# dubhater/vapoursynth-mvtools

Measured on AMD Instinct MI355X. Metric: MDegrain3 cfg3 fps (Super+Analyse+Degrain end-to-end), higher is better.
Workload: dtype u16; 1 GPU; 4K YUV420P16 Degrain3 blksize=16 overlap=8 pel=2; batches_in_flight=2

## Files before the change

### vapoursynth-mvtools_amd/csrc/mvx_analyse.hip

```cpp
#include <stdarg.h>
#include <stdlib.h>

#include <algorithm>
#include "mvx_analyse_kernel.h"
#include "mvx_analyse_fast.h"
#include "mvx_analyse_spec.h"
int mvx_analyse_launch_spec_u8(const AParams &P, const ASpecLaunch &S);
int mvx_analyse_launch_spec_u16(const AParams &P, const ASpecLaunch &S);


static thread_local char g_err[512];
void mvx_set_error(const char *fmt, ...) {
    va_list ap;
    va_start(ap, fmt);
    vsnprintf(g_err, sizeof(g_err), fmt, ap);
    va_end(ap);
}
extern "C" __attribute__((visibility("default"))) const char *mvx_last_error(void) { return g_err; }

struct MvxDebug {
    int general = 0;
    int cpw1 = 0;
    int spec = 1;
    int team = -1;
// ... 278 lines not shown
        int fMaxBlkX = 0;
        for (int i = 0; i < P.nLevels; i++) if (P.lv[i].nBlkX > fMaxBlkX) fMaxBlkX = P.lv[i].nBlkX;
        const int fBins = 1024;
        int fNeed = fRow + fMaxBlkX * 16;
        if (fNeed < fRow + fBins * 4) fNeed = fRow + fBins * 4;
        const bool stripShape8 = P.bps == 1 && P.blkX == 8 && P.chroma && (P.ovX == 4 || P.ovX == 0) && P.shadow[1] != 0;
        const bool uvOrLumaOnly = P.chroma ? P.shadow[1] != 0 : true;
        const bool stripShape16 = P.bps == 1 && P.blkX == 16 && uvOrLumaOnly && (P.ovX == 8 || P.ovX == 0);
        const bool stripShape = (P.bps == 2 && (P.blkX == 16 || (MVX_STRIP32 && P.blkX == 32)) && uvOrLumaOnly && (P.ovX == P.blkX / 2 || (P.blkX == 16 && P.ovX == 0))) || stripShape8 || stripShape16;
        const int sStrip = (P.bps == 2 && P.blkX == 16) ? 2 * 24 * 128  : (P.bps == 2 && MVX_STRIP32 && P.blkX == 32) ? (P.blkX + P.blkX / 2) * 128 : (P.bps == 1 && P.blkX == 16) ? 24 * 64 : 0;
        const int sSrc = stripShape8 ? 16 + 768 : fRow < sStrip ? sStrip : fRow;
        int sNeed = 0, sTabMax = 0;
        for (int i = 0; i < P.nLevels; i++) {
            const bool smallest = i == P.nLevels - 1;
            const int st = smallest ? (P.nLevels == 1 ? P.searchType : P.searchTypeCoarse) : (i == 0 ? P.searchType : P.searchTypeCoarse);
            const int tabB = (st == SearchHex2 ? SPEC_SLOTS_HEX : SPEC_SLOTS_EXH) * SPEC_STRIDE;
            const int need = sSrc + ((P.lv[i].nBlkX * 8 + 15) & ~15) + tabB;
            if (need > sNeed) sNeed = need;
            if (tabB > sTabMax) sTabMax = tabB;
        }
        if (sNeed < sSrc + fBins * 4) sNeed = sSrc + fBins * 4;
        const int teamShared = (64 + fMaxBlkX * 8 + 255) & ~255;
        const int teamPerWave = ((sSrc + sTabMax < sSrc + fBins * 4 ? sSrc + fBins * 4 : sSrc + sTabMax) + 255) & ~255;
        auto teamThatFits = [&](int team) {
            if (team == 1 || team > 8) team = 0;
            while (team > 1 && teamShared + teamPerWave * team > 160 * 1024) team--;
            return team > 1 ? team : 0;
        };
        const bool teamAnyShape = g_dbg.spec == 1 && g_dbg.team < 0 && teamThatFits(mvx_team_default(njobs, simds, false, P.bps)) > 0;
        const bool useSpec = g_dbg.spec != 0 && (stripShape || g_dbg.spec >= 2 || teamAnyShape);
        const bool useSpecStrips = useSpec && g_dbg.spec != 3 && stripShape;
        int sTab = 0, sRow = fRow;
        if (useSpec) {
            sRow = sSrc;
            sTab = sSrc + ((fMaxBlkX * 8 + 15) & ~15);
            fNeed = sNeed;
        }
        const int perChain = (fNeed + 255) & ~255;
        auto have = [&](int k) {
            if (P.bps == 2 && P.blkX == 8) return k == 1 || k == 2 || k == 4;
            if (P.bps == 2 && P.blkX == 32) return k >= 1 && k <= 3;
            return k >= 1 && k <= 4;
        };
        int k = njobs > 3 * simds ? 4 : njobs > 2 * simds ? 3 : njobs > simds ? 2 : 1;
        if (useSpecStrips && k > 2) k = 2;
        while (k > 1 && (!have(k) || (long long)perChain * 4 * k > 160 * 1024)) k--;
        if ((long long)perChain * 4 * k <= 160 * 1024) {
            const int cpw = useSpecStrips ? 4 : 4 * k;
            int syncEvery = k >= 2 ? (P.bps == 2 ? 32 : 256) : 0;
            if (useSpecStrips) syncEvery = (stripShape8 || stripShape16) ? 0 : 128;
            const int flags = MVX_FAST_XCD_REMAP | ((P.shadow[1] != 0 && P.chroma) ? MVX_FAST_UV : 0) | (g_dbg.spec == 2 ? MVX_FAST_NOSPEC : 0) | (g_dbg.spec == 3 ? MVX_FAST_NOSTRIP : 0);
            const ALaunch L = { njobs, 0, useSpec ? sRow : fRow, useSpec ? sRow : fRow, fBins, fNeed, simds, cpw, k, syncEvery, k, flags, st, a->dP, S.d };
            int rc;
            const int specSide = (P.blkX == 16 && P.ovX == 0) ? 1 : 0;
            const int team = useSpec ? teamThatFits(g_dbg.team >= 0 ? g_dbg.team : mvx_team_default(njobs, simds, useSpecStrips, P.bps)) : 0;
            if (team) {
                ALaunch TL = L;
                TL.ldsRow = teamShared; TL.ldsNeed = teamPerWave; TL.ldsHist = sRow; TL.syncEvery = 0; TL.fast = 2; TL.cpw = 1;
                const ASpecLaunch SL = { TL, sRow, team, specSide };
                rc = P.bps == 1 ? mvx_analyse_launch_spec_u8(P, SL) : mvx_analyse_launch_spec_u16(P, SL);
                if (rc == MVX_OK) return finish(2, team, 0, 3);
                if (rc != 1) return rc;
            }
            if (useSpec) { const ASpecLaunch SL = { L, sTab, 0, specSide }; rc = P.bps == 1 ? mvx_analyse_launch_spec_u8(P, SL) : mvx_analyse_launch_spec_u16(P, SL); }
            else rc = P.bps == 1 ? mvx_analyse_launch_fast_u8(P, L) : mvx_analyse_launch_fast_u16(P, L);
            if (rc == MVX_OK) return finish(k, cpw, syncEvery, useSpec ? 2 : 0);
            if (rc != 1) return rc;
        }
    }
    const bool specialised = P.dctmode == 0 && P.xr == 2 && P.yr == 2 && P.blkX == P.blkY && (P.blkX == 16 || P.blkX == 8 || (P.blkX == 32 && P.bps == 2));
    int cpw = g_dbg.cpw1 ? 1 : 4, wpe = 1;
    if (specialised && !g_dbg.cpw1 && njobs > simds) {
        if (P.bps == 1 && (P.blkX == 8 || P.blkX == 16)) wpe = 2;
        if (P.bps == 1 && P.blkX == 8 && njobs > 2 * simds) wpe = 3;
        if (P.bps == 2 && (P.blkX == 16 || P.blkX == 8 || P.blkX == 32)) { wpe = 2; cpw = 8; }
    }
    int srcBytes = P.blkX * P.blkY * P.bps;
    if (P.chroma) srcBytes += 2 * (P.blkX / P.xr) * (P.blkY / P.yr) * P.bps;
    int ldsRow = (srcBytes + 15) & ~15;
    int maxBlkX = 0;
    for (int i = 0; i < P.nLevels; i++) if (P.lv[i].nBlkX > maxBlkX) maxBlkX = P.lv[i].nBlkX;
    const int histBins = 1024;
    const int ldsHist = ldsRow + maxBlkX * 16;
    int ldsBytes = ldsHist + histBins * 4;
    if (ldsBytes > 160 * 1024) { mvx_set_error("mvx_analyse_frames: frame too wide for the LDS row buffer"); return MVX_E_ARG; }
    const int ldsNeed = ldsBytes;
    if (ldsBytes < 33 * 1024) ldsBytes = 33 * 1024;
    while (cpw > 1 && (long long)((ldsNeed + 255) & ~255) * cpw > 160 * 1024) {
        cpw = cpw == 8 ? 4 : 1;
        if (wpe == 3) wpe = 2;
        if (P.bps == 2) wpe = 1;
    }
    const int syncEvery = wpe >= 2 ? 256 : 0;
    const ALaunch L = { njobs, ldsBytes, ldsRow, ldsHist, histBins, ldsNeed, simds, cpw, wpe, syncEvery, 0, 0, st, a->dP, S.d };
    bool off32 = true;
    for (int i = 0; i < P.nLevels; i++)
        if ((long long)P.lv[i].pel * P.lv[i].pel * P.lv[i].pstride[0] >= 0xffffffffLL || (long long)P.lv[i].pel * P.lv[i].pel * P.lv[i].pstride[1] >= 0xffffffffLL) off32 = false;
    int rc = (P.dctmode != 0 || !off32) ? 1 : P.bps == 1 ? mvx_analyse_launch_u8(P, L) : mvx_analyse_launch_u16(P, L);
    if (rc == 1) rc = mvx_analyse_launch_any(P, L);
    if (rc) return rc;
    return finish(0, cpw, syncEvery, 0);
}


struct mvx_recalculate {
    mvx_analysis_data ad, adOut, old;
    AParams P;
// ... 165 lines not shown
```

### vapoursynth-mvtools_amd/csrc/mvx_analyse_spec.h

```cpp
#pragma once
#include <type_traits>
#include "mvx_analyse_fast.h"

#define SPEC_TB 32
#define SPEC_STRIDE (SPEC_TB * 8 + 8)
#define SPEC_SLOTS_HEX 19
#define SPEC_SLOTS_EXH 29
#define MVX_FAST_NOSTRIP 8
#define MVX_FAST_NOSPEC 4

constexpr int SPEC_SW3 = 12;
#ifdef MVX_SPEC_PROF
#define SPROF_N 20
static __device__ unsigned long long g_specprof[SPROF_N];
#define SPROF(i) do { const long long t1_ = (long long)__builtin_amdgcn_s_memtime(); asm volatile("s_waitcnt lgkmcnt(0)" : : "s"(t1_) : "memory"); sprof[i] += t1_ - sprofT; sprofT = t1_; } while (0)
#else
#define SPROF(i) ((void)0)
#endif
#ifdef MVX_SPEC_PROF
#define SPEC_PROF_DUMP_() do { if (l == 0 && chain == 5 && S.role == 1) for (int i = 0; i < SPROF_N; i++) g_specprof[i] = (unsigned long long)S.sprof[i]; } while (0)
#else
#define SPEC_PROF_DUMP_() ((void)0)
#endif
#ifdef MVX_SPEC_STATS
// ... 86 lines not shown
        const unsigned idx = (unsigned)((ax & m) | ((ay & m) << logPel));
        return idx * pstrideC + (unsigned)(ay >> logPel) * pitchC + (unsigned)(ax >> logPel) * BPS;
    }
    template <int LOGG, int WMAX> __device__ __forceinline__ void pass_start(int s, int bx0, int vx, int vy, int vyc, unsigned &oA, unsigned &oB) const {
        typedef PG<LOGG, WMAX> Q;
        const int rowA = s >> G::LLOGC, xbA = (s & (Q::CA - 1)) * G::LCB, rowB = s >> G::UVLOGC, xbB = (s & (Q::CB - 1)) * G::UVCB;
        oA = luma_off_at(bx0, vx, vy) + (unsigned)rowA * pitchY + (unsigned)xbA;
        oB = 2 * chroma_off_at(bx0, vx, vyc) + (unsigned)rowB * 2 * pitchC + (unsigned)xbB;
    }
    template <int LOGG, int WMAX> __device__ __forceinline__ v4u pass_issue(Pass<LOGG, WMAX> &T, int piece) const {
        typedef PG<LOGG, WMAX> Q;
        v4u v;
        if (piece < Q::NA) { v = F::template ld_ref<G::LCB>(refY + T.curA); T.curA += (unsigned)(Q::GG >> G::LLOGC) * pitchY; asm volatile("" : "+v"(T.curA) : : "memory"); }
        else { v = F::template ld_ref<G::UVCB>(refUV + T.curB); T.curB += (unsigned)(Q::GG >> G::UVLOGC) * 2 * pitchC; asm volatile("" : "+v"(T.curB) : : "memory"); }
        return v;
    }
    template <int LOGG, int WMAX> __device__ __forceinline__ void pass_prime(Pass<LOGG, WMAX> &T, unsigned oA, unsigned oB) const {
        typedef PG<LOGG, WMAX> Q;
        T.curA = oA; T.curB = oB;
#pragma unroll
        for (int k = 0; k < Q::W; k++) T.r[k] = pass_issue(T, k);
    }
    template <int LOGG, int WMAX, bool REFILL = true> __device__ __forceinline__ void pass_run(Pass<LOGG, WMAX> &T, int s, unsigned nA, unsigned nB) const {
        typedef PG<LOGG, WMAX> Q;
        const int rowA = s >> G::LLOGC, xbA = (s & (Q::CA - 1)) * G::LCB, rowB = s >> G::UVLOGC, xbB = (s & (Q::CB - 1)) * G::UVCB;
        const lds_u8 *spA = lds + rowA * G::LROWB + xbA, *spB = lds + G::UOFF + rowB * G::UVROWB + xbB;
        constexpr int lstepA = (Q::GG >> G::LLOGC) * G::LROWB, lstepB = (Q::GG >> G::UVLOGC) * G::UVROWB;
        auto src_piece = [&](int k) { return k < Q::NA ? F::template lds_piece<G::LCB>(spA + k * lstepA) : F::template lds_piece<G::UVCB>(spB + (k - Q::NA) * lstepB); };
        constexpr int D = MVX_SRC_AHEAD < Q::NT ? MVX_SRC_AHEAD : Q::NT;
        v4u a[D];
#pragma unroll
        for (int k = 0; k < D; k++) a[k] = src_piece(k);
        unsigned aL = 0, aC = 0;
#pragma unroll
        for (int k = 0; k < Q::NT; k++) {
            const v4u cur = a[k % D];
            if (k + D < Q::NT) a[k % D] = src_piece(k + D);
            if (k < Q::NA) aL = F::template sad_regs<G::LCB>(cur, T.r[k % Q::W], aL);
            else aC = F::template sad_regs<G::UVCB>(cur, T.r[k % Q::W], aC);
            asm volatile("" : "+v"(aL), "+v"(aC) : : "memory");
            const int kk = k + Q::W;
            if (kk == Q::NT) { T.curA = nA; T.curB = nB; }
            if (REFILL || kk < Q::NT) T.r[k % Q::W] = pass_issue(T, kk % Q::NT);
        }
        T.aL = aL; T.aC = aC;
    }

#ifndef MVX_STRIP32
#define MVX_STRIP32 0
#endif
    static constexpr bool STRIP_OK = (BPS == 2 && (BW == 16 || (MVX_STRIP32 && BW == 32))) || (BPS == 1 && BW == 16);
    static constexpr int COLB = BPS == 2 ? 16 : 8, ROWB = 8 * COLB;
    static constexpr int HC = STRIP_OK ? BW / 16 : 1, SW_BLOCKS = 8 / HC - 1, LPB = 2 * HC, LPC = SW_BLOCKS * LPB;
    static_assert(!SIDE || (STRIP_OK && HC == 1), "blocks side by side: 16x16 row passes only");
    static constexpr int pickSW(int nt, int w) { return w <= 1 ? 1 : (w <= nt && nt % w == 0) ? w : pickSW(nt, w - 1); }
    static constexpr int SNA = BW, SNB = UV ? BW / 2 : 0, SNT = SNA + SNB, SW = pickSW(SNT, (BW == 32 && SWIN > 12) ? 12 : SWIN), S_UV = SNA * ROWB, SSTG = SNT / 8;
    struct StripPass { v4u r[SW]; unsigned curA, curB, aL, aC; };
    __device__ __forceinline__ v4u strip_issue(StripPass &T, int piece) const {
        v4u v;
        if (piece < SNA) { v = F::template ld_ref<COLB>(refY + T.curA); T.curA += pitchY; asm volatile("" : "+v"(T.curA) : : "memory"); }
        else { v = F::template ld_ref<COLB>(refUV + T.curB); T.curB += 2 * pitchC; asm volatile("" : "+v"(T.curB) : : "memory"); }
        return v;
    }
    __device__ __forceinline__ void strip_prime(StripPass &T, unsigned oA, unsigned oB) const {
        T.curA = oA; T.curB = oB;
#pragma unroll
        for (int k = 0; k < SW; k++) T.r[k] = strip_issue(T, k);
    }
    template <bool REFILL> __device__ __forceinline__ void strip_run(StripPass &T, int p, unsigned nA, unsigned nB, int bufOff = 0) const {
        const lds_u8 *sp = lds + bufOff + p * COLB;
        auto src_piece = [&](int k) { return F::template lds_piece<COLB>(sp + (k < SNA ? k * ROWB : S_UV + (k - SNA) * ROWB)); };
        constexpr int D = MVX_SRC_AHEAD;
        v4u a[D];
#pragma unroll
        for (int k = 0; k < D; k++) a[k] = src_piece(k);
        unsigned aL = 0, aC = 0;
#pragma unroll
        for (int k = 0; k < SNT; k++) {
            const v4u cur = a[k % D];
            if (k + D < SNT) a[k % D] = src_piece(k + D);
            if (k < SNA) aL = F::template sad_regs<COLB>(cur, T.r[k % SW], aL);
            else aC = F::template sad_regs<COLB>(cur, T.r[k % SW], aC);
            asm volatile("" : "+v"(aL), "+v"(aC) : : "memory");
            const int kk = k + SW;
            if (kk == SNT) { T.curA = nA; T.curB = nB; }
            if (REFILL || kk < SNT) T.r[k % SW] = strip_issue(T, kk % SNT);
        }
        T.aL = aL; T.aC = aC;
    }
    static constexpr bool STRIP8_OK = UV && BPS == 1 && BW == 8;
    static constexpr int W8_BLOCKS = 15, R8A = 8, R8B = 4, R8T = R8A + R8B;
    struct Strip8 { v4u r[R8T]; unsigned curA, curB; unsigned aL[4], aC[4]; };
    __device__ __forceinline__ v4u strip8_issue(Strip8 &T, int piece) const {
        v4u v;
        if (piece < R8A) { v = F::template ld_ref<16>(refY + T.curA); T.curA += pitchY; asm volatile("" : "+v"(T.curA) : : "memory"); }
        else { v = F::template ld_ref<16>(refUV + T.curB); T.curB += 2 * pitchC; asm volatile("" : "+v"(T.curB) : : "memory"); }
        return v;
    }
    __device__ __forceinline__ void strip8_prime(Strip8 &T, unsigned oA, unsigned oB) const {
        T.curA = oA; T.curB = oB;
#pragma unroll
        for (int k = 0; k < R8T; k++) T.r[k] = strip8_issue(T, k);
    }
    static constexpr int S8_BASE = 16;
    template <bool REFILL> __device__ __forceinline__ void strip8_run(Strip8 &T, int srcA, int srcB, int shA, int shB, unsigned nA, unsigned nB) const {
        const lds_u8 *spA = lds + S8_BASE + srcA, *spB = lds + S8_BASE + srcB;
        auto src_piece = [&](int k) {
            const LDS_AS unsigned *q = (const LDS_AS unsigned *)((k < R8A ? spA : spB) + k * 64);
            return v4u{q[0], q[1], q[2], q[3]};
        };
        unsigned aL0 = 0, aL1 = 0, aL2 = 0, aL3 = 0, aC0 = 0, aC1 = 0, aC2 = 0, aC3 = 0;
        v4u a = src_piece(0);
#pragma unroll
        for (int k = 0; k < R8T; k++) {
            const v4u cur = a;
            if (k + 1 < R8T) a = src_piece(k + 1);
            const v4u rr = T.r[k];
            if (k < R8A) { aL0 = __builtin_amdgcn_sad_u8(cur[0], rr[0], aL0); aL1 = __builtin_amdgcn_sad_u8(cur[1], rr[1], aL1); aL2 = __builtin_amdgcn_sad_u8(cur[2], rr[2], aL2); aL3 = __builtin_amdgcn_sad_u8(cur[3], rr[3], aL3); }
            else { aC0 = __builtin_amdgcn_sad_u8(cur[0], rr[0], aC0); aC1 = __builtin_amdgcn_sad_u8(cur[1], rr[1], aC1); aC2 = __builtin_amdgcn_sad_u8(cur[2], rr[2], aC2); aC3 = __builtin_amdgcn_sad_u8(cur[3], rr[3], aC3); }
            asm volatile("" : "+v"(aL0), "+v"(aC0) : : "memory");
            if (k == 0) { T.curA = nA; T.curB = nB; }
            if (REFILL) T.r[k] = strip8_issue(T, k);
        }
        auto rot = [](unsigned &a0, unsigned &a1, unsigned &a2, unsigned &a3, int sh) {
            const bool o = sh & 1, t = sh & 2;
            const unsigned b0 = o ? a1 : a0, b1 = o ? a2 : a1, b2 = o ? a3 : a2, b3 = o ? a0 : a3;
            a0 = t ? b2 : b0; a1 = t ? b3 : b1; a2 = t ? b0 : b2; a3 = t ? b1 : b3;
        };
        rot(aL0, aL1, aL2, aL3, shA); rot(aC0, aC1, aC2, aC3, shB);
        T.aL[0] = aL0; T.aL[1] = aL1; T.aL[2] = aL2; T.aL[3] = aL3; T.aC[0] = aC0; T.aC[1] = aC1; T.aC[2] = aC2; T.aC[3] = aC3;
    }
    __device__ __forceinline__ static void pat_delta(bool hex, int idx, int &dx, int &dy) {
        dx = 0; dy = 0;
        if (hex) {
            if (idx < 6) { dx = tab8(HEX2X >> 8, idx & 7); dy = tab8(HEX2Y >> 8, idx & 7); }
            else if (idx < 14) { dx = tab8(PACK8(0, 0, -1, 1, -1, -1, 1, 1), idx - 6); dy = tab8(PACK8(-1, 1, 0, 0, -1, 1, -1, 1), idx - 6); }
        } else {
            if (idx < 8) { dx = tab8(PACK8(0, 0, -1, 1, -1, -1, 1, 1), idx); dy = tab8(PACK8(-1, 1, 0, 0, -1, 1, -1, 1), idx); }
            else if (idx < 16) { dx = tab8(PACK8(-1, -1, 0, 0, 1, 1, -2, 2), idx - 8); dy = tab8(PACK8(-2, 2, -2, 2, -2, 2, -1, -1), idx - 8); }
            else if (idx < 24) { dx = tab8(PACK8(-2, 2, -2, 2, -2, -2, 2, 2), idx - 16); dy = tab8(PACK8(0, 0, 1, 1, -2, 2, -2, 2), idx - 16); }
        }
    }

    __device__ __forceinline__ void search_level_spec(int lvl, int globalX, int globalY, GL_AS const GVec *coarse, int coarseBlkX, int coarseBlkY, int coarseLogPel, int syncEvery, bool specEnabled, bool stripEnabled) {
// ... 9 lines not shown
        pitchY = (unsigned)uni((int)P.pitch[0]); pitchC = (unsigned)uni((int)P.pitch[1]); pstrideY = (unsigned)uni((int)L.pstride[0]); pstrideC = (unsigned)uni((int)L.pstride[1]);
        shadowY = (unsigned)uni((int)P.shadow[0]);
        srcUV = uptr(J.src[1] + P.shadow[1] + 2 * L.off[1]); refUV = uptr((J.ref[1] ? J.ref[1] : J.src[1]) + P.shadow[1] + 2 * L.off[1]);
        unsigned char *rec = (unsigned char *)(unsigned long long)uni((long long)(unsigned long long)(J.blob + L.blobOff));
        vectors = (GL_AS GVec *)(rec + 4);
        if (l == 0 && (!TEAM || role == 0)) *(int *)rec = 4 + nBlkX * nBlkY * 16;
        const bool smallestPlane = lvl == P.nLevels - 1;
        if constexpr (TEAM) {
            if (role == 0 && l < 8) ctl[l] = 0;
            this->interpolate(coarse, coarseBlkX, coarseBlkY, coarseLogPel, l + 64 * role, 64 * nw);
        } else this->interpolate(coarse, coarseBlkX, coarseBlkY, coarseLogPel);
        __builtin_amdgcn_fence(__ATOMIC_RELEASE, "workgroup");
        __builtin_amdgcn_fence(__ATOMIC_ACQUIRE, "workgroup");
        __builtin_amdgcn_s_barrier();

        if (smallestPlane) { searchType = P.nLevels == 1 ? P.searchType : P.searchTypeCoarse; nSearchParam = P.nLevels == 1 ? P.nPelSearch : P.nSearchParam; }
        else { searchType = lvl == 0 ? P.searchType : P.searchTypeCoarse; nSearchParam = lvl == 0 ? P.nPelSearch : P.nSearchParam; }
        searchType = uni(searchType); nSearchParam = uni(nSearchParam);
        fieldShift = uni(lvl == 0 ? J.fieldShift : 0);
        badSAD = uni(P.badSAD); badrange = uni(P.badrange); badcount = 0;
        gmvx = pel * globalX; gmvy = pel * globalY + fieldShift;
        int nLambdaLevel = P.lambda / (pel * pel);
        const int nScale = 1 << lvl;
        if (P.plevel == 1) nLambdaLevel = nLambdaLevel * nScale;
        else if (P.plevel == 2) nLambdaLevel = nLambdaLevel * nScale * nScale;
        nLambdaLevel = uni(nLambdaLevel);
        penaltyZero = uni(P.pzero); pglobal = uni(P.global ? P.pglobal : P.pzero); penaltyNew = uni(P.pnew); LSAD = uni((long long)P.lsad);
        const int stepX = uni(P.blkX - P.ovX), stepY = uni(P.blkY - P.ovY);
        const int hps = hpad >> lvl, vps = vpad >> lvl;
        const bool meander = uni(P.meander) != 0;
        LDS_AS v2u *rowbuf = (LDS_AS v2u *)(TEAM ? shRow : lds + ldsRow);
        lds_u8 *tab = TEAM ? lds + ldsTab : lds + ldsRow + ((nBlkX * 8 + 15) & ~15);
        this->pf_setup();
        SPROF(8);
        auto lambda_of = [&](int predSad) {
            const double scale = (double)LSAD / (double)(LSAD + (long long)(predSad >> 1));
            return (int)(long long)((double)(long long)nLambdaLevel * scale * scale);
        };
        const bool hexLevel = searchType == SearchHex2;
        const bool specLevel = specEnabled && !smallestPlane;
        int rdx = 0, rdy = 0;
        if (hexLevel) {
            const int g = l >> 2;
            if (g < 6) { rdx = tab8(HEX2X >> 8, g & 7); rdy = tab8(HEX2Y >> 8, g & 7); }
            else if (g < 14) { rdx = tab8(PACK8(0, 0, -1, 1, -1, -1, 1, 1), g - 6); rdy = tab8(PACK8(-1, 1, 0, 0, -1, 1, -1, 1), g - 6); }
        } else {
            const int g = l >> 1, k = g < 8 ? g : g - 8;
            if (g < 8) { rdx = tab8(PACK8(0, 0, -1, 1, -1, -1, 1, 1), k); rdy = tab8(PACK8(-1, 1, 0, 0, -1, 1, -1, 1), k); }
            else if (g < 16) { rdx = tab8(PACK8(-1, -1, 0, 0, 1, 1, -2, 2), k); rdy = tab8(PACK8(-2, 2, -2, 2, -2, 2, -1, -1), k); }
            else if (g < 24) { rdx = tab8(PACK8(-2, 2, -2, 2, -2, -2, 2, 2), k - 8); rdy = tab8(PACK8(0, 0, 1, 1, -2, 2, -2, 2), k - 8); }
        }
        unsigned sPat = 0, bPat0 = 0, bPat1 = 0;
        {
            const bool side8 = STRIP8_OK && stepX == BW;
            constexpr bool side16 = SIDE;
            const int gb = side8 ? l >> 3 : STRIP8_OK ? (l >= 45 ? 3 : l >= 30 ? 2 : l >= 15 ? 1 : 0) : side16 ? min(l >> 3, 3) : min(l / LPC, 3);
            for (int q = 0; q < 8; q++) {
                int dx, dy;
                if (q < 4) { pat_delta(hexLevel, STRIP8_OK ? q * 16 + (l >> 2) : q * 8 + (l >> 3), dx, dy); sPat |= (unsigned)((dx & 15) | ((dy & 15) << 4)) << (8 * q); }
                pat_delta(hexLevel, q * (side8 ? 8 : 4) + gb, dx, dy);
                const unsigned b = (unsigned)((dx & 15) | ((dy & 15) << 4)) << (8 * (q & 3));
                if (q < 4) bPat0 |= b; else bPat1 |= b;
            }
        }
#ifdef MVX_SPEC_STATS
        unsigned long long st0 = 0, st1 = 0, st2 = 0, st3 = 0, st4 = 0, st5 = 0, st6 = 0, st7 = 0;
#endif

        int prevX = 0, prevY = 0, prevSad = 0;
        int syncCount = 0;
        if (syncEvery > 0 && syncEvery < 32) syncEvery = 32;
        int Gc = 0;
        const int nGrpRow = (nBlkX + SPEC_TB - 1) / SPEC_TB;
        for (int blky = 0; blky < nBlkY; blky++) {
            const bool fwd = (blky & 1) == 0 || !meander;
            const int dir = fwd ? 1 : -1;
            y0 = vpad + stepY * blky;
            nDyMax = (ph - y0 - BW - vpad + vps) << logPel;
            nDyMin = -((y0 - vpad + vps) << logPel);
            if constexpr (TEAM) gmvy = this->clipy(gmvy);
            const bool specRow = specLevel && blky > 0;
            const int ngrp = (nBlkX + 63) >> 6;
            for (int gi = 0; gi < ngrp; gi++) {
                const int grp = fwd ? gi : ngrp - 1 - gi;
                const int c0 = grp << 6, c = c0 + l;
                const bool in = c < nBlkX;
                const int ncol = min(64, nBlkX - c0);
                v4u bOut = {0, 0, 0, 0};
                for (int hi = 0; hi < 2; hi++) {
                    const int h = fwd ? hi : 1 - hi;
                    const int lo = h * SPEC_TB, hiE = min(lo + SPEC_TB, ncol);
                    if (lo >= ncol) continue;
                    const int myG = Gc++;
                    bool teamHeld = false;
                    if constexpr (TEAM) {
                        if (uni(myG % nw) != role) {
                            gmvx = team_advance(gmvx, c0, lo, hiE, fwd, stepX, hps);
                            continue;
                        }
                        if (specRow) {
                            const int j = (c0 >> 5) + h;
                            const bool fwdPrev = ((blky - 1) & 1) == 0 || !meander;
                            auto idxPrev = [&](int jj) { return fwdPrev ? jj : nGrpRow - 1 - jj; };
                            int need = (blky - 1) * nGrpRow + idxPrev(j) + 1;
                            if (blky == nBlkY - 1) { const int j2 = j + dir; if (j2 >= 0 && j2 < nGrpRow) need = max(need, (blky - 1) * nGrpRow + idxPrev(j2) + 1); }
                            SPROF(7);
                            team_wait_ge(need);
                            SPROF(16);
                        }
                    }
                    SPROF(7);
                    if (syncEvery && (syncCount++ & ((syncEvery >> 5) - 1)) == 0) __builtin_amdgcn_s_barrier();
                    SPROF(0);
                    const bool act = l >= lo && l < hiE;
                    unsigned long long okmask = 0, flagmask = 0;
                    int rX = 0, rY = 0, rSad = 0;
                    int pkU = 0, pkAh = 0, pkH = 0, pkG = 0;
                    int lam = 0;
                    bool staged2G = false;
                    int lamG = 0, pBestG = 0, pkWG = 0;
                    int gEndX = gmvx;
                    if (specRow) {
                        const int xs = stepX * c;
                        const int dxMin = -((xs + hps) << logPel), dxMax1 = ((pw - xs - hpad - BW - hpad + hps) << logPel) - 1;
                        auto cx = [&](int v) { return min(max(v, dxMin), dxMax1); };
                        auto cy = [&](int v) { return min(max(v, nDyMin), nDyMax - 1); };
                        v4u bSelf = {0, 0, 0, 0}, bBelow = {0, 0, 0, 0};
                        unsigned upPk = 0;
                        if (in) {
                            bSelf = this->ld_batch(&vectors[blky * nBlkX + c]);
                            const int cb = c + dir;
                            if (blky < nBlkY - 1 && cb >= 0 && cb < nBlkX) bBelow = this->ld_batch(&vectors[(blky + 1) * nBlkX + cb]);
                            upPk = rowbuf[c][0];
                        }
                        lam = in ? lambda_of((int)bSelf[2]) : 0;
                        const int ux = cx(upx((int)upPk)), uy = cy(upy((int)upPk));
                        pkU = pk(ux, uy);
                        const bool aheadCol = fwd ? c < nBlkX - 1 : c > 0;
                        const bool useBelow = blky < nBlkY - 1 && aheadCol;
                        int ahx = 0, ahy = fieldShift;
                        if (useBelow) { ahx = (int)bBelow[0]; ahy = (int)bBelow[1]; }
                        else if (aheadCol && in) { const v2u t = rowbuf[c + dir]; ahx = upx((int)t[0]); ahy = upy((int)t[0]); }
                        const int ax = cx(ahx), ay = cy(ahy);
                        pkAh = pk(ax, ay);
                        const int hx = cx((int)bSelf[0]), hy = cy((int)bSelf[1]);
                        pkH = pk(hx, hy);
                        gmvy = this->clipy(gmvy);
                        if (__ballot(act && cx(gmvx) != gmvx) == 0) pkG = pk(gmvx, gmvy);
                        else {
                            for (int i = 0; i < hiE - lo; i++) {
                                const int li = fwd ? lo + i : hiE - 1 - i;
                                const int xb = stepX * (c0 + li);
                                gmvx = min(max(gmvx, -((xb + hps) << logPel)), ((pw - xb - hpad - BW - hpad + hps) << logPel) - 1);
                                pkG = l == li ? pk(gmvx, gmvy) : pkG;
                            }
                        }
                        gEndX = gmvx;

                        const int ti8L = (l & (SPEC_TB - 1)) * 8;
                        auto rd = [&](int slot) { return *(const LDS_AS v2u *)(tab + slot * SPEC_STRIDE + ti8L); };
                        auto tot = [&](const v2u &t) { return (int)t[0] + (chroma ? (int)t[1] : 0); };
                        auto md = [&](int vx, int vy) {
                            const unsigned dx = (unsigned)(hx - vx), dy = (unsigned)(hy - vy);
                            const int dist = (int)(dx * dx + dy * dy);
                            return (int)(((long long)lam * dist) >> 8);
// ... 21 lines not shown
#pragma unroll
                                for (int k = 0; k < 14; k++) tt[k] = rd(k);
                                if (nSearchParam > 1) {
#pragma unroll
                                    for (int k = 0; k < 6; k++) {
                                        const int vx = wx + tab8(HEX2X >> 8, k), vy = wy + tab8(HEX2Y >> 8, k);
                                        won = won || (vok(vx, vy) && cnew(vx, vy, tt[k]) < best);
                                    }
                                }
#pragma unroll
                                for (int k = 0; k < 8; k++) {
                                    const int vx = wx + tab8(PACK8(0, 0, -1, 1, -1, -1, 1, 1), k), vy = wy + tab8(PACK8(-1, 1, 0, 0, -1, 1, -1, 1), k);
                                    const v2u t = tt[6 + k];
                                    const int cc = cnew(vx, vy, t);
                                    if (vok(vx, vy) && cc < best) { best = cc; bx = vx; by = vy; bs = tot(t); }
                                }
                            } else {
#pragma unroll 1
                                for (int k0 = 0; k0 < 24; k0 += 8) {
                                    v2u tt[8];
#pragma unroll
                                    for (int k = 0; k < 8; k++) tt[k] = rd(k0 + k);
#pragma unroll
                                    for (int k = 0; k < 8; k++) {
                                        int dx, dy;
                                        if (k0 == 0) { dx = tab8(PACK8(0, 0, -1, 1, -1, -1, 1, 1), k); dy = tab8(PACK8(-1, 1, 0, 0, -1, 1, -1, 1), k); }
                                        else if (k0 == 8) { dx = tab8(PACK8(-1, -1, 0, 0, 1, 1, -2, 2), k); dy = tab8(PACK8(-2, 2, -2, 2, -2, 2, -1, -1), k); }
                                        else { dx = tab8(PACK8(-2, 2, -2, 2, -2, -2, 2, 2), k); dy = tab8(PACK8(0, 0, 1, 1, -2, 2, -2, 2), k); }
                                        const int vx = wx + dx, vy = wy + dy;
                                        const v2u t = tt[k];
                                        const int cc = cnew(vx, vy, t);
                                        if (vok(vx, vy) && cc < best) { best = cc; bx = vx; by = vy; bs = tot(t); }
                                    }
                                }
                            }
                            return won;
                        };
                        bool staged2 = false;
                        int pBest = 0, pX_ = 0, pY_ = fieldShift, pSad = 0;

                        const int nb = hiE - lo;
                        const bool lumaStrips = STRIP_OK && !UV && !chroma && stripEnabled && stepX == (SIDE ? BW : BW / 2);
                        const bool streamed = (chroma && (hexLevel ? STREAM_HEX : STREAM_EXH)) || lumaStrips;
                        if (streamed) {
                            const int pkZ = pk(0, fieldShift);
                            const int slotUp = hexLevel ? 14 : 24, slotZ = hexLevel ? 16 : 26;
                            unsigned long long pbMask = __ballot(act), p3Mask = 0;

                            SPROF(1);
                            if constexpr (STRIP_OK) {
                                constexpr bool side = SIDE;
                                if (stripEnabled && stepX == (side ? BW : BW / 2) && (UV ? chroma != 0 : chroma == 0)) {
                                    constexpr int TC = side ? 2 : HC, SWB = side ? 4 : SW_BLOCKS, LPCr = SWB * LPB;
                                    const int nw = (nb + SWB - 1) / SWB;
                                    const int npat = hexLevel ? 14 : 24;
                                    pbMask = 0;
                                    staged2 = true;
                                    unsigned stripW = 0;
                                    int pkW = 0;
                                    int lq = l;
                                    asm volatile("" : "+v"(lq));
                                    int gS, pS, gB, rB, mB, hB;
                                    bool tail, idleB;
                                    auto roles = [&]() {
                                        lq = l;
                                        asm volatile("" : "+v"(lq));
                                        gS = lq >> 3; pS = lq & 7;
                                        gB = side ? min(lq >> 3, 3) : min(lq / LPC, 3);
                                        rB = side ? (lq & 7) : lq >= 4 * LPC ? (lq - 4 * LPC) % LPC : lq - LPC * gB; mB = rB / LPB; hB = rB % LPB;
                                        tail = lq >= 56; idleB = lq >= 4 * LPCr;
                                    };
                                    roles();
                                    auto w_cand = [&](int st, int w, int q, int &slot, int &colW, bool &stripLane, int &srcCol, unsigned &oA, unsigned &oB) {
                                        const int f = lo + SWB * w, L = min(SWB, hiE - f);
                                        const int bxf = hpad + stepX * (c0 + f);
                                        const bool stripWin = st == 2 && ((stripW >> w) & 1);
                                        const int meB = min(mB, L - 1), colB = f + meB;
                                        int bU = 0, bAh = 0, bG = 0, bH = 0, bW = 0;
                                        if (st == 1) {
                                            bU = __builtin_amdgcn_ds_bpermute(colB << 2, pkU); bAh = __builtin_amdgcn_ds_bpermute(colB << 2, pkAh);
                                            bG = __builtin_amdgcn_ds_bpermute(colB << 2, pkG); bH = __builtin_amdgcn_ds_bpermute(colB << 2, pkH);
                                        } else if (!stripWin) bW = __builtin_amdgcn_ds_bpermute(colB << 2, pkW);
                                        if (stripWin || (st == 1 && tail)) {
                                            const int p = st == 1 ? pS : pS, g = gS;
                                            int vx, vy, vyc;
                                            if (st == 1) { vx = 0; vy = fieldShift; vyc = 0; slot = slotZ; }
                                            else {
                                                const int sW = __builtin_amdgcn_readlane(pkW, f);
                                                const int idx = q * 8 + g;
                                                const int dd = (int)(sPat >> (8 * q)), dx = (dd << 28) >> 28, dy = (dd << 24) >> 28;
                                                vx = upx(sW) + dx; vy = upy(sW) + dy; vyc = vy;
                                                slot = idx < npat ? idx : -1;
                                            }
                                            const int pe = min(p, TC * (L - 1) + 2 * HC - 1) * COLB;
                                            if ((p % TC != 0) | (p / TC >= L)) slot = -1;
                                            colW = f + p / TC; stripLane = true; srcCol = p;
                                            oA = luma_off_at(bxf, vx, vy) + (unsigned)pe;
                                            oB = 2 * chroma_off_at(bxf, vx, vyc) + (unsigned)pe;
                                        } else {
                                            const int me = meB, col = colB;
                                            int base, dx = 0, dy = 0;
                                            if (st == 1) {
                                                base = gB == 0 ? bU : gB == 1 ? bAh : gB == 2 ? bG : bH;
                                                slot = gB == 0 ? slotUp : gB == 1 ? slotUp + 1 : slotZ + gB - 1;
                                            } else {
                                                base = bW;
// ... 56 lines not shown
                                            SPROF(2);
                                            if (more) w_cand(st, wn, qn, slotN, colN, stripN, srcN, nA, nB);
                                            SPROF(11);
                                            if (q == 0) {
                                                __builtin_amdgcn_wave_barrier();
                                                stage_store();
                                                if (wi + 1 < wTo) stage_issue(widx(wi + 1), sbuf ^ 1);
                                                __builtin_amdgcn_wave_barrier();
                                            }
                                            SPROF(12);
                                            if (more) strip_run<true>(T, srcCol, nA, nB, SDMA ? sbuf * SBUF : 0); else strip_run<false>(T, srcCol, 0, 0, SDMA ? sbuf * SBUF : 0);
                                            SPROF(13);
                                            unsigned sL = T.aL + (unsigned)__builtin_amdgcn_update_dpp(0, (int)T.aL, 0x101, 0xf, 0xf, true), sC = T.aC + (unsigned)__builtin_amdgcn_update_dpp(0, (int)T.aC, 0x101, 0xf, 0xf, true);
                                            unsigned hL = T.aL + (unsigned)__builtin_amdgcn_update_dpp(0, (int)T.aL, 0xB1, 0xf, 0xf, true), hC = T.aC + (unsigned)__builtin_amdgcn_update_dpp(0, (int)T.aC, 0xB1, 0xf, 0xf, true);
                                            if (HC == 2) {
                                                sL += (unsigned)__builtin_amdgcn_update_dpp(0, (int)sL, 0x102, 0xf, 0xf, true); sC += (unsigned)__builtin_amdgcn_update_dpp(0, (int)sC, 0x102, 0xf, 0xf, true);
                                                hL += (unsigned)__builtin_amdgcn_update_dpp(0, (int)hL, 0x4E, 0xf, 0xf, true); hC += (unsigned)__builtin_amdgcn_update_dpp(0, (int)hC, 0x4E, 0xf, 0xf, true);
                                            }
                                            if (slot >= 0) *(LDS_AS v2u *)(tab + slot * SPEC_STRIDE + (colW & (SPEC_TB - 1)) * 8) = v2u{stripLane ? sL : hL, stripLane ? sC : hC};
                                            SPROF(14);
#ifdef MVX_SPEC_PROF
                                            sprof[15] += 1;
#endif
                                            if (!more) break;
                                            if (SDMA && win != wi) sbuf ^= 1;
                                            w = wn; wi = win; q = qn; slot = slotN; colW = colN; stripLane = stripN; srcCol = srcN;
                                        }
                                        __builtin_amdgcn_wave_barrier();
                                    };
                                    run_stage(1, 0, nw);
                                    a2_pred(pBest, pX_, pY_, pSad);
                                    pkW = pk(pX_, pY_);
                                    {
                                        const bool ok2 = (pX_ - 2 >= dxMin) & (pX_ + 2 <= dxMax1) & (pY_ - 2 >= nDyMin) & (pY_ + 2 < nDyMax);
                                        for (int w = 0; w < nw; w++) {
                                            const int f = lo + SWB * w, e = min(f + SWB, hiE);
                                            const bool inw = (l >= f) & (l < e);
                                            const int w0 = __builtin_amdgcn_readlane(pkW, f);
                                            if (e - f >= 2 && __ballot(inw & ((pkW != w0) | !ok2)) == 0) stripW |= 1u << w;
#ifdef MVX_SPEC_STATS
                                            if ((stripW >> w) & 1) st4 += 1;
                                            else { st5 += 1; st6 += __builtin_popcountll(__ballot(inw & (pkW != w0))); if (__ballot(inw & (pkW != w0)) == 0) st7 += 1; }
#endif
                                        }
                                    }
                                    run_stage(2, 0, nw);
                                }
                            }

                            if constexpr (STRIP8_OK) {
                                auto rows8 = [&](auto DS2) {
                                    constexpr bool ds2 = decltype(DS2)::value;
                                    const int wmax = ds2 ? 8 : W8_BLOCKS;
                                    const int nw = (nb + wmax - 1) / wmax, WL = (nb + nw - 1) / nw;
                                    const int npat = hexLevel ? 14 : 24;
                                    pbMask = 0;
                                    staged2 = true;
                                    unsigned stripW = 0;
                                    int pkW = 0;
                                    int lq, gS, qS, gB, mB;
                                    bool tail;
                                    auto roles = [&]() {
                                        lq = l;
                                        asm volatile("" : "+v"(lq));
                                        gS = lq >> 2; qS = lq & 3;
                                        if (ds2) { gB = lq >> 3; mB = lq & 7; }
                                        else { gB = min(lq / W8_BLOCKS, 3); mB = lq >= 60 ? lq - 60 : lq - W8_BLOCKS * gB; }
                                        tail = lq >= 60;
                                    };
                                    roles();
                                    auto w_cand = [&](int st, int w, int q, int &slot, int &colW, int &nwr, int &srcA, int &srcB, int &shA, int &shB, unsigned &oA, unsigned &oB) {
                                        const int f = lo + WL * w, L = min(WL, hiE - f);
                                        const int bxf = hpad + stepX * (c0 + f);
                                        const bool stripWin = st == 2 && ((stripW >> w) & 1);
                                        const int meB = min(mB, L - 1), colB = f + meB;
                                        int bU = 0, bAh = 0, bG = 0, bH = 0, bW = 0;
                                        if (st == 1) {
                                            bU = __builtin_amdgcn_ds_bpermute(colB << 2, pkU); bAh = __builtin_amdgcn_ds_bpermute(colB << 2, pkAh);
                                            bG = __builtin_amdgcn_ds_bpermute(colB << 2, pkG); bH = __builtin_amdgcn_ds_bpermute(colB << 2, pkH);
                                        } else if (!stripWin) bW = __builtin_amdgcn_ds_bpermute(colB << 2, pkW);
                                        const int nd = ds2 ? 2 * L : L + 1;
                                        if (stripWin || (st == 1 && tail)) {
                                            int vx, vy, vyc;
                                            if (st == 1) { vx = 0; vy = fieldShift; vyc = 0; slot = slotZ; }
                                            else {
                                                const int sW = __builtin_amdgcn_readlane(pkW, f);
                                                const int idx = q * 16 + gS;
                                                const int dd = (int)(sPat >> (8 * q)), dx = (dd << 28) >> 28, dy = (dd << 24) >> 28;
                                                vx = upx(sW) + dx; vy = upy(sW) + dy; vyc = vy;
                                                slot = idx < npat ? idx : -1;
                                            }
                                            const int qe = min(qS, (nd - 1) >> 2), d0 = min(4 * qe, nd - 4);
                                            nwr = ds2 ? max(0, min(2, L - 2 * qS)) : max(0, min(4, L - 4 * qS));
                                            if (nwr == 0) slot = -1;
                                            colW = f + (ds2 ? 2 : 4) * qS; srcA = srcB = d0 * 4; shA = shB = 4 * qe - d0;
                                            oA = luma_off_at(bxf, vx, vy) + (unsigned)(d0 * 4);
                                            oB = 2 * chroma_off_at(bxf, vx, vyc) + (unsigned)(d0 * 4);
                                        } else {
                                            int base, dx = 0, dy = 0;
                                            if (st == 1) {
                                                base = gB == 0 ? bU : gB == 1 ? bAh : gB == 2 ? bG : bH;
                                                slot = gB == 0 ? slotUp : gB == 1 ? slotUp + 1 : slotZ + gB - 1;
                                            } else {
                                                base = bW;
                                                const int ci = q * (ds2 ? 8 : 4) + gB;
                                                const int dd = (int)((q < 4 ? bPat0 : bPat1) >> (8 * (q & 3)));
// ... 29 lines not shown
                                    auto run_stage = [&](int st) {
                                        int wi = 0, w = widx(0), q = 0;
                                        Strip8 T;
                                        int slot, colW, nwr, srcA, srcB, shA, shB; unsigned oA, oB;
                                        roles();
                                        w_cand(st, w, q, slot, colW, nwr, srcA, srcB, shA, shB, oA, oB);
                                        strip8_prime(T, oA, oB);
                                        stage_issue(w);
                                        for (;;) {
                                            roles();
                                            int wn = w, qn = q + 1, win = wi;
                                            if (qn >= npass(st, w)) { qn = 0; win = wi + 1; wn = widx(win); }
                                            const bool more = win < nw;
                                            int slotN = -1, colN = 0, nwrN = 0, srcAN = 0, srcBN = 0, shAN = 0, shBN = 0; unsigned nA = 0, nB = 0;
                                            if (more) w_cand(st, wn, qn, slotN, colN, nwrN, srcAN, srcBN, shAN, shBN, nA, nB);
                                            if (q == 0) {
                                                __builtin_amdgcn_wave_barrier();
                                                stage_store();
                                                if (wi + 1 < nw) stage_issue(widx(wi + 1));
                                                __builtin_amdgcn_wave_barrier();
                                            }
                                            if (more) strip8_run<true>(T, srcA, srcB, shA, shB, nA, nB); else strip8_run<false>(T, srcA, srcB, shA, shB, 0, 0);
                                            const unsigned xL = (unsigned)__builtin_amdgcn_update_dpp(0, (int)T.aL[0], 0x101, 0xf, 0xf, true), xC = (unsigned)__builtin_amdgcn_update_dpp(0, (int)T.aC[0], 0x101, 0xf, 0xf, true);
                                            if (slot >= 0) {
                                                lds_u8 *tp = tab + slot * SPEC_STRIDE;
                                                *(LDS_AS v2u *)(tp + (colW & (SPEC_TB - 1)) * 8) = v2u{T.aL[0] + T.aL[1], T.aC[0] + T.aC[1]};
                                                if (ds2) {
                                                    if (nwr > 1) *(LDS_AS v2u *)(tp + ((colW + 1) & (SPEC_TB - 1)) * 8) = v2u{T.aL[2] + T.aL[3], T.aC[2] + T.aC[3]};
                                                } else {
                                                    if (nwr > 1) *(LDS_AS v2u *)(tp + ((colW + 1) & (SPEC_TB - 1)) * 8) = v2u{T.aL[1] + T.aL[2], T.aC[1] + T.aC[2]};
                                                    if (nwr > 2) *(LDS_AS v2u *)(tp + ((colW + 2) & (SPEC_TB - 1)) * 8) = v2u{T.aL[2] + T.aL[3], T.aC[2] + T.aC[3]};
                                                    if (nwr > 3) *(LDS_AS v2u *)(tp + ((colW + 3) & (SPEC_TB - 1)) * 8) = v2u{T.aL[3] + xL, T.aC[3] + xC};
                                                }
                                            }
                                            if (!more) break;
                                            w = wn; wi = win; q = qn; slot = slotN; colW = colN; nwr = nwrN; srcA = srcAN; srcB = srcBN; shA = shAN; shB = shBN;
                                        }
                                        __builtin_amdgcn_wave_barrier();
                                    };
                                    run_stage(1);
                                    a2_pred(pBest, pX_, pY_, pSad);
                                    pkW = pk(pX_, pY_);
                                    {
                                        const bool ok2 = (pX_ - 2 >= dxMin) & (pX_ + 2 <= dxMax1) & (pY_ - 2 >= nDyMin) & (pY_ + 2 < nDyMax);
                                        for (int w = 0; w < nw; w++) {
                                            const int f = lo + WL * w, e = min(f + WL, hiE);
                                            const bool inw = (l >= f) & (l < e);
                                            const int w0 = __builtin_amdgcn_readlane(pkW, f);
                                            if (e - f >= 2 && __ballot(inw & ((pkW != w0) | !ok2)) == 0) stripW |= 1u << w;
                                        }
                                    }
                                    run_stage(2);
                                };
                                if (stripEnabled && nb >= 3) {
                                    if (stepX == BW / 2) rows8(std::false_type());
                                    else if (stepX == BW) rows8(std::true_type());
                                }
                            }

                            SPROF(2);
                            auto r_cand = [&](int li, int &bx0, int &vx, int &vy, int &vyc) {
                                bx0 = hpad + stepX * (c0 + li);
                                const int xMax = (pw - bx0 - BW - hpad + hps) << logPel, xMin = -((bx0 - hpad + hps) << logPel);
                                const int sU = __builtin_amdgcn_readlane(pkU, li), sAh = __builtin_amdgcn_readlane(pkAh, li);
                                int base;
                                if (hexLevel) base = (l >> 2) == 15 ? sAh : sU;
                                else {
                                    const int g = l >> 1;
                                    const int sH = __builtin_amdgcn_readlane(pkH, li), sG = __builtin_amdgcn_readlane(pkG, li);
                                    base = g == 25 ? sAh : g == 26 ? pkZ : g == 27 ? sG : g == 28 ? sH : sU;
                                }
                                const int cxv = upx(base), cyv = upy(base);
                                const int tx = cxv + rdx, ty = cyv + rdy;
                                const bool ok = (tx >= xMin) & (ty >= nDyMin) & (tx < xMax) & (ty < nDyMax);
                                vx = ok ? tx : cxv; vy = ok ? ty : cyv;
                                vyc = (!hexLevel && (l >> 1) == 26) ? 0 : vy;
                            };
                            auto p_cand = [&](int li, bool ahFirst, int &bx0, int &vx, int &vy, int &vyc) {
                                bx0 = hpad + stepX * (c0 + li);
                                const int g = l >> LOGGP;
                                const int sH = __builtin_amdgcn_readlane(pkH, li), sG = __builtin_amdgcn_readlane(pkG, li), sAh = __builtin_amdgcn_readlane(pkAh, li);
                                const int base = g == 1 ? sG : g == 2 ? sH : ahFirst ? sAh : pkZ;
                                vx = upx(base); vy = upy(base); vyc = ((g == 1) | (g == 2) | ahFirst) ? vy : 0;
                            };
                            auto first_of = [](unsigned long long m) { return (int)__builtin_ctzll(m); };
                            if (pbMask) {
                                A4x32 pf[G::NPF];
                                unsigned long long m = pbMask;
                                int li = first_of(m);
                                m &= m - 1;
                                this->pf_issue(hpad + stepX * (c0 + li), y0, pf);
                                if (hexLevel) {
                                    if constexpr (STREAM_HEX) {
                                        Pass<2, 12> R; Pass<LOGGP, 4> Z;
                                        const int sR = l & 3, sZ = l & ((1 << LOGGP) - 1);
                                        {
                                            int bx0, vx, vy, vyc; unsigned oA, oB;
                                            r_cand(li, bx0, vx, vy, vyc); this->template pass_start<2, 12>(sR, bx0, vx, vy, vyc, oA, oB); this->template pass_prime<2, 12>(R, oA, oB);
                                            p_cand(li, false, bx0, vx, vy, vyc); this->template pass_start<LOGGP, 4>(sZ, bx0, vx, vy, vyc, oA, oB); this->template pass_prime<LOGGP, 4>(Z, oA, oB);
                                        }
                                        for (;;) {
                                            const bool more = m != 0;
                                            const int lin = more ? first_of(m) : li;
                                            m &= m - 1;
                                            __builtin_amdgcn_wave_barrier();
                                            this->pf_store(pf);
                                            if (more) this->pf_issue(hpad + stepX * (c0 + lin), y0, pf);
                                            int bx0, vx, vy, vyc; unsigned nA = 0, nB = 0, mA = 0, mB = 0;
                                            if (more) {
                                                r_cand(lin, bx0, vx, vy, vyc); this->template pass_start<2, 12>(sR, bx0, vx, vy, vyc, nA, nB);
// ... 409 lines not shown
```

### vapoursynth-mvtools_amd/csrc/mvx_analyse_spec_u8.hip

```cpp
#include "mvx_analyse_kernel.h"
#include "mvx_analyse_spec.h"
int mvx_analyse_launch_spec_u8(const AParams &P, const ASpecLaunch &S) {
    const int k = S.L.fast;
    if (S.side && P.blkX == 16) {
        if (S.team) return launch_analyse_spec_team<1, 16, 2, 8, true>(S);
        return launch_analyse_spec<1, 16, 2, 8, true>(S);
    }
    if (S.team) {
        if (P.blkX == 8) return launch_analyse_spec_team<1, 8, 2, 8>(S);
        if (P.blkX == 16) return launch_analyse_spec_team<1, 16, 2, 8>(S);
        return 1;
    }
    if (P.blkX == 8) {
        if (k == 4) return launch_analyse_spec<1, 8, 4, 16>(S);
        if (k == 3) return launch_analyse_spec<1, 8, 3, 12>(S);
        if (k == 2) return launch_analyse_spec<1, 8, 2, 8>(S);
        if (k == 1) return launch_analyse_spec<1, 8, 1, 4>(S);
    }
    if (P.blkX == 16) {
        if (k == 4) return launch_analyse_spec<1, 16, 4, 16>(S);
        if (k == 3) return launch_analyse_spec<1, 16, 3, 12>(S);
        if (k == 2) return launch_analyse_spec<1, 16, 2, 8>(S);
        if (k == 1) return launch_analyse_spec<1, 16, 1, 4>(S);
    }
    return 1;
}
```

Baseline: 931.0 fps.

## Add side-by-side 8-bit 8x8 strip path and size column groups by strip window

Enables the side-by-side (non-overlapped) strip specialisation for 8-bit 8x8 blocks with chroma. The column group length is now derived from the strip window size (GT/FR) rather than a fixed 32/64, and the barrier cadence is recomputed in groups. This aims to avoid partial windows and wasted lanes in non-overlapped configs, at the cost of more template instantiations and changed group and sync bookkeeping. The benchmark is u16 with overlap 8, so the new side path does not apply here, though the GT changes still compile into the u16 kernels.

```diff
diff --git a/vapoursynth-mvtools_amd/csrc/mvx_analyse.hip b/vapoursynth-mvtools_amd/csrc/mvx_analyse.hip
--- a/vapoursynth-mvtools_amd/csrc/mvx_analyse.hip
+++ b/vapoursynth-mvtools_amd/csrc/mvx_analyse.hip
@@ -354,7 +354,7 @@
             const int flags = MVX_FAST_XCD_REMAP | ((P.shadow[1] != 0 && P.chroma) ? MVX_FAST_UV : 0) | (g_dbg.spec == 2 ? MVX_FAST_NOSPEC : 0) | (g_dbg.spec == 3 ? MVX_FAST_NOSTRIP : 0);
             const ALaunch L = { njobs, 0, useSpec ? sRow : fRow, useSpec ? sRow : fRow, fBins, fNeed, simds, cpw, k, syncEvery, k, flags, st, a->dP, S.d };
             int rc;
-            const int specSide = (P.blkX == 16 && P.ovX == 0) ? 1 : 0;
+            const int specSide = ((P.blkX == 16 || stripShape8) && P.ovX == 0) ? 1 : 0;
             const int team = useSpec ? teamThatFits(g_dbg.team >= 0 ? g_dbg.team : mvx_team_default(njobs, simds, useSpecStrips, P.bps)) : 0;
             if (team) {
                 ALaunch TL = L;
diff --git a/vapoursynth-mvtools_amd/csrc/mvx_analyse_spec.h b/vapoursynth-mvtools_amd/csrc/mvx_analyse_spec.h
--- a/vapoursynth-mvtools_amd/csrc/mvx_analyse_spec.h
+++ b/vapoursynth-mvtools_amd/csrc/mvx_analyse_spec.h
@@ -162,7 +162,6 @@
     static constexpr bool STRIP_OK = (BPS == 2 && (BW == 16 || (MVX_STRIP32 && BW == 32))) || (BPS == 1 && BW == 16);
     static constexpr int COLB = BPS == 2 ? 16 : 8, ROWB = 8 * COLB;
     static constexpr int HC = STRIP_OK ? BW / 16 : 1, SW_BLOCKS = 8 / HC - 1, LPB = 2 * HC, LPC = SW_BLOCKS * LPB;
-    static_assert(!SIDE || (STRIP_OK && HC == 1), "blocks side by side: 16x16 row passes only");
     static constexpr int pickSW(int nt, int w) { return w <= 1 ? 1 : (w <= nt && nt % w == 0) ? w : pickSW(nt, w - 1); }
     static constexpr int SNA = BW, SNB = UV ? BW / 2 : 0, SNT = SNA + SNB, SW = pickSW(SNT, (BW == 32 && SWIN > 12) ? 12 : SWIN), S_UV = SNA * ROWB, SSTG = SNT / 8;
     struct StripPass { v4u r[SW]; unsigned curA, curB, aL, aC; };
@@ -200,6 +199,10 @@
     }
     static constexpr bool STRIP8_OK = UV && BPS == 1 && BW == 8;
     static constexpr int W8_BLOCKS = 15, R8A = 8, R8B = 4, R8T = R8A + R8B;
+    static_assert(!SIDE || (STRIP_OK && HC == 1) || STRIP8_OK, "blocks side by side: the 16x16 and the 8-bit 8x8 row passes only");
+    static constexpr int WBLK = STRIP_OK ? (SIDE ? 4 : SW_BLOCKS) : STRIP8_OK ? (SIDE ? 8 : W8_BLOCKS) : SPEC_TB;
+    static constexpr int GT = SPEC_TB / WBLK * WBLK, FR = 2 * GT;
+    static_assert(GT >= 1 && GT <= SPEC_TB && FR <= 64, "a group fits the table, a frame the wave");
     struct Strip8 { v4u r[R8T]; unsigned curA, curB; unsigned aL[4], aC[4]; };
     __device__ __forceinline__ v4u strip8_issue(Strip8 &T, int piece) const {
         v4u v;
@@ -315,7 +318,7 @@
         }
         unsigned sPat = 0, bPat0 = 0, bPat1 = 0;
         {
-            const bool side8 = STRIP8_OK && stepX == BW;
+            constexpr bool side8 = STRIP8_OK && SIDE;
             constexpr bool side16 = SIDE;
             const int gb = side8 ? l >> 3 : STRIP8_OK ? (l >= 45 ? 3 : l >= 30 ? 2 : l >= 15 ? 1 : 0) : side16 ? min(l >> 3, 3) : min(l / LPC, 3);
             for (int q = 0; q < 8; q++) {
@@ -331,10 +334,10 @@
 #endif
 
         int prevX = 0, prevY = 0, prevSad = 0;
-        int syncCount = 0;
-        if (syncEvery > 0 && syncEvery < 32) syncEvery = 32;
+        const int syncGroups = syncEvery > 0 ? max(1, (syncEvery + GT / 2) / GT) : 0;
+        int syncCount = syncGroups - 1;
         int Gc = 0;
-        const int nGrpRow = (nBlkX + SPEC_TB - 1) / SPEC_TB;
+        const int nGrpRow = (nBlkX + GT - 1) / GT;
         for (int blky = 0; blky < nBlkY; blky++) {
             const bool fwd = (blky & 1) == 0 || !meander;
             const int dir = fwd ? 1 : -1;
@@ -343,16 +346,16 @@
             nDyMin = -((y0 - vpad + vps) << logPel);
             if constexpr (TEAM) gmvy = this->clipy(gmvy);
             const bool specRow = specLevel && blky > 0;
-            const int ngrp = (nBlkX + 63) >> 6;
+            const int ngrp = (nBlkX + FR - 1) / FR;
             for (int gi = 0; gi < ngrp; gi++) {
                 const int grp = fwd ? gi : ngrp - 1 - gi;
-                const int c0 = grp << 6, c = c0 + l;
-                const bool in = c < nBlkX;
-                const int ncol = min(64, nBlkX - c0);
+                const int c0 = grp * FR, c = c0 + l;
+                const int ncol = min(FR, nBlkX - c0);
+                const bool in = l < ncol;
                 v4u bOut = {0, 0, 0, 0};
                 for (int hi = 0; hi < 2; hi++) {
                     const int h = fwd ? hi : 1 - hi;
-                    const int lo = h * SPEC_TB, hiE = min(lo + SPEC_TB, ncol);
+                    const int lo = h * GT, hiE = min(lo + GT, ncol);
                     if (lo >= ncol) continue;
                     const int myG = Gc++;
                     bool teamHeld = false;
@@ -362,7 +365,7 @@
                             continue;
                         }
                         if (specRow) {
-                            const int j = (c0 >> 5) + h;
+                            const int j = 2 * grp + h;
                             const bool fwdPrev = ((blky - 1) & 1) == 0 || !meander;
                             auto idxPrev = [&](int jj) { return fwdPrev ? jj : nGrpRow - 1 - jj; };
                             int need = (blky - 1) * nGrpRow + idxPrev(j) + 1;
@@ -373,7 +376,7 @@
                         }
                     }
                     SPROF(7);
-                    if (syncEvery && (syncCount++ & ((syncEvery >> 5) - 1)) == 0) __builtin_amdgcn_s_barrier();
+                    if (syncGroups && ++syncCount == syncGroups) { __builtin_amdgcn_s_barrier(); syncCount = 0; }
                     SPROF(0);
                     const bool act = l >= lo && l < hiE;
                     unsigned long long okmask = 0, flagmask = 0;
@@ -501,6 +504,7 @@
                                 constexpr bool side = SIDE;
                                 if (stripEnabled && stepX == (side ? BW : BW / 2) && (UV ? chroma != 0 : chroma == 0)) {
                                     constexpr int TC = side ? 2 : HC, SWB = side ? 4 : SW_BLOCKS, LPCr = SWB * LPB;
+                                    static_assert(SWB == WBLK, "the group length is counted in these windows");
                                     const int nw = (nb + SWB - 1) / SWB;
                                     const int npat = hexLevel ? 14 : 24;
                                     pbMask = 0;
@@ -663,6 +667,7 @@
                                 auto rows8 = [&](auto DS2) {
                                     constexpr bool ds2 = decltype(DS2)::value;
                                     const int wmax = ds2 ? 8 : W8_BLOCKS;
+                                    static_assert((ds2 ? 8 : W8_BLOCKS) == WBLK, "the group length is counted in these windows");
                                     const int nw = (nb + wmax - 1) / wmax, WL = (nb + nw - 1) / nw;
                                     const int npat = hexLevel ? 14 : 24;
                                     pbMask = 0;
@@ -798,10 +803,7 @@
                                     }
                                     run_stage(2);
                                 };
-                                if (stripEnabled && nb >= 3) {
-                                    if (stepX == BW / 2) rows8(std::false_type());
-                                    else if (stepX == BW) rows8(std::true_type());
-                                }
+                                if (stripEnabled && nb >= 3 && stepX == (SIDE ? BW : BW / 2)) rows8(std::integral_constant<bool, SIDE>());
                             }
 
                             SPROF(2);
diff --git a/vapoursynth-mvtools_amd/csrc/mvx_analyse_spec_u8.hip b/vapoursynth-mvtools_amd/csrc/mvx_analyse_spec_u8.hip
--- a/vapoursynth-mvtools_amd/csrc/mvx_analyse_spec_u8.hip
+++ b/vapoursynth-mvtools_amd/csrc/mvx_analyse_spec_u8.hip
@@ -5,6 +5,13 @@
     if (S.side && P.blkX == 16) {
         if (S.team) return launch_analyse_spec_team<1, 16, 2, 8, true>(S);
         return launch_analyse_spec<1, 16, 2, 8, true>(S);
+    }
+    if (S.side && P.blkX == 8 && (S.L.flags & MVX_FAST_UV)) {
+        if (S.team) return launch_analyse_spec_team_uv<1, 8, 2, 8, true, true>(S);
+        if (k == 4) return launch_analyse_spec_uv<1, 8, 4, 16, true, true>(S);
+        if (k == 3) return launch_analyse_spec_uv<1, 8, 3, 12, true, true>(S);
+        if (k == 2) return launch_analyse_spec_uv<1, 8, 2, 8, true, true>(S);
+        if (k == 1) return launch_analyse_spec_uv<1, 8, 1, 4, true, true>(S);
     }
     if (S.team) {
         if (P.blkX == 8) return launch_analyse_spec_team<1, 8, 2, 8>(S);
```

Result: faster. 965.4 fps, median of 6 (+3.7%).
